# ug93tad/singa

Measured on AMD Instinct MI355X. Metric: images/sec (whole node) ResNet-50 bf16 training, higher is better.
Workload: dtype bf16; 1 GPU; model=ResNet-50, global_batch=1024, image=224, parallelism=dp1, exec=hipgraph, optimizer=SGD momentum 0.9 wd 1e-4, deterministic=True

## Files before the change

### singa_amd/autograd.py

```python
from __future__ import annotations

import builtins as _b
import math
import os
import sys
import threading
import types
import heapq
import weakref
from collections import Counter, deque
from typing import Callable, Dict, Iterator, List, Optional, Sequence, Tuple

import numpy as np
import torch

from . import memory as _mem
from . import tensor as _tensor
from .ops import functional as F
from .ops import glue as G
from .ops import native as N
from .tensor import Tensor

_TLS = threading.local()

# ... 790 lines not shown
            del dx._sg_absorbed
            dx = AccReplace(dx)
        elif acc is not None and (dx is acc or (isinstance(acc, F.LAZY_GRADS) and acc.value is not None
                                                and dx is acc.value)):
            dx = ACC_INPLACE
        res = [dx, ACCUMULATED if tgt is not None else dw]
        if self.has_bias:
            res.append(ACCUMULATED if tb is not None else db)
        return tuple(res)


class BatchNorm2d(Operator):

    def __init__(self, running_mean: torch.Tensor, running_var: torch.Tensor, momentum: float = 0.1,
                 eps: float = 1e-5, relu: bool = False, has_residual: bool = False, name=None,
                 colsum: bool = False):
        super().__init__(name)
        self.rm, self.rv = running_mean, running_var
        self.momentum, self.eps = momentum, eps
        self.relu, self.has_residual = relu, has_residual
        self.colsum = colsum

    def forward(self, x, gamma, beta, res=None):
        want = self.requires_grad and self.relu and (self.has_residual or (F.BN_WDOT and _training()))
        y, st = F.batchnorm_fwd(x, gamma, beta, self.rm, self.rv, _training(), self.momentum, self.eps, self.relu,
                                res, want_mask=want, want_colsum=self.colsum and self.requires_grad)
        if self.requires_grad:
            self.x, self.gamma, self.st = x, gamma, st
            self.beta = beta if F.BN_WDOT else None
            self.y = y if (want and st.mask is None) else None
        return y

    def backward(self, dy):
        tg, tb = self.grad_target(1), self.grad_target(2)
        dx, dg, db, dres = F.batchnorm_bwd(self.x, dy, self.gamma, self.st, self.y, need_dres=self.has_residual,
                                           relu=self.relu, dg_out=tg, db_out=tb, beta=getattr(self, "beta", None),
                                           lazy_dres=True)
        self.x = self.y = self.st = self.beta = None
        out = [dx, ACCUMULATED if tg is not None else dg, ACCUMULATED if tb is not None else db]
        if self.has_residual:
            out.append(dres)
# ... 31 lines not shown
        pre = getattr(dout, "_sg_gsum", None)
        if pre is not None and pre[1] is st.mask:
            g, gws = dout, pre[0]
            del dout._sg_gsum
        else:
            g, gws = F.bnres_masksum(dout, st.mask)
        prod = self.src[0][0] if self.src else None
        prod2 = None
        if (isinstance(prod, BatchNorm2d) and prod.relu and not prod.has_residual and F.BN_WDOT
                and getattr(prod, "st", None) is not None and prod.st.mask is not None
                and getattr(prod, "beta", None) is not None and (getattr(self, "sole", None) or {}).get(0, False)
                and self.needs_grad(0)):
            prod2 = (prod.st.mask, prod.gamma, prod.beta)
        tw, tg, tb = self.grad_target(1), self.grad_target(2), self.grad_target(3)
        cs = getattr(getattr(prod, "st", None), "colsum", None) if isinstance(prod, BatchNorm2d) else None
        dy, dw, dg, db = F.bnres_bwd(g, gws, y, w, st, gamma, dw_out=tw, dg_out=tg, db_out=tb, prod2=prod2, cs=cs)
        if tw is not None:
            _WGRAD_EPOCH[id(self.params[1])] = GRAD_EPOCH[0]
        g._sg_fresh = True
        acc = lambda tgt, v: ACCUMULATED if tgt is not None else v
        return dy, acc(tw, dw), acc(tg, dg), acc(tb, db), g


class ConvBNDualAddReLU(Operator):

    wants_sole = True

    def __init__(self, bn3, bnd, stride: int, name=None):
        super().__init__(name)
        self.p3 = (bn3.running_mean.data, bn3.running_var.data, 1.0 - bn3.momentum, bn3.eps)
        self.pd = (bnd.running_mean.data, bnd.running_var.data, 1.0 - bnd.momentum, bnd.eps)
# ... 31 lines not shown
        if pre is not None and pre[1] is st3.mask:
            g, gws = dout, pre[0]
            del dout._sg_gsum
        else:
            g, gws = F.bnres_masksum(dout, st3.mask)
        prod = self.src[0][0] if self.src else None
        prod2 = None
        if (isinstance(prod, BatchNorm2d) and prod.relu and not prod.has_residual and F.BN_WDOT
                and getattr(prod, "st", None) is not None and prod.st.mask is not None
                and getattr(prod, "beta", None) is not None and (getattr(self, "sole", None) or {}).get(0, False)
                and self.needs_grad(0)):
            prod2 = (prod.st.mask, prod.gamma, prod.beta)
        cs = getattr(getattr(prod, "st", None), "colsum", None) if isinstance(prod, BatchNorm2d) else None
        t = [self.grad_target(i) for i in (1, 2, 3, 5, 6, 7)]
        dy, dw3, dg3, db3 = F.bnres_bwd(g, gws, y, w3, st3, g3, dw_out=t[0], dg_out=t[1], db_out=t[2], prod2=prod2,
                                        cs=cs)
        dxs, dwd, dgd, dbd = F.bnres_bwd(g, gws, xs, wd, std, gd, dw_out=t[3], dg_out=t[4], db_out=t[5])
        for i, tg in ((1, t[0]), (5, t[3])):
            if tg is not None:
                _WGRAD_EPOCH[id(self.params[i])] = GRAD_EPOCH[0]
        dx = None
        if self.needs_grad(4):
            dx = dxs if self.stride == 1 else (F.StridedGrad(dxs, self.stride, xshape) if F.STRIDED_LAZY
                                               else F.strided_place(dxs, xshape, self.stride))
        acc = lambda tgt, v: ACCUMULATED if tgt is not None else v
        return (dy, acc(t[0], dw3), acc(t[1], dg3), acc(t[2], db3), dx, acc(t[3], dwd), acc(t[4], dgd),
                acc(t[5], dbd))


class DualBNAddReLU(Operator):

    def __init__(self, bn1, bn2, name=None):
# ... 1138 lines not shown
```

### singa_amd/csrc/bindings.cpp

```cpp
#include <hip/hip_runtime.h>
#include <pybind11/pybind11.h>
#include <pybind11/stl.h>
#include <stdint.h>
#include <stdexcept>
#include <string>
#include <vector>

namespace py = pybind11;
typedef uintptr_t P;
#define V(x) ((void*)(x))
#define CV(x) ((const void*)(x))
#define S(x) ((hipStream_t)(x))

extern "C" {
void sg_unary_fwd(int, const void*, void*, int64_t, int, float, hipStream_t);
void sg_unary_bwd(int, const void*, const void*, const void*, void*, int64_t, int, float, hipStream_t);
void sg_add_act(const void*, const void*, void*, int64_t, int, float, float, int, hipStream_t);
void sg_relu_bwd_from_y(const void*, const void*, void*, int64_t, int, hipStream_t);
void sg_mask_bits_apply(const void*, const void*, void*, int64_t, hipStream_t);
void sg_zero_ranges(void*, const void*, int, hipStream_t);
void sg_cast(const void*, int, void*, int, int64_t, hipStream_t);
void sg_dropout_fwd(const void*, void*, void*, int64_t, int, float, uint64_t, uint64_t, const void*, hipStream_t);
void sg_dropout_bwd(const void*, const void*, void*, int64_t, int, float, hipStream_t);
void sg_rand_fill(void*, int64_t, int, int, float, float, uint64_t, uint64_t, hipStream_t);
// ... 100 lines not shown
int sg_conv3x3_enabled();
void sg_bnres_wgrad(const void*, const void*, void*, int, int, int, hipStream_t);
void sg_bnres_dgrad(const void*, const void*, const void*, const void*, void*, int, int, int, void*, const void*,
                    hipStream_t);
void sg_bnres_coef(const void*, const void*, const void*, const void*, const void*, const void*, int, int, int, void*,
                   void*, void*, void*, void*, hipStream_t);
void sg_bnres_combine(const void*, const void*, const void*, const void*, int, const void*, const void*, int, int,
                      void*, void*, void*, void*, const void*, const void*, float, hipStream_t);
void sg_bnres_masksum(const void*, const void*, void*, void*, int64_t, int, hipStream_t);
void sg_set_dgrad_mask_out(int);
void sg_bn_apply_cs(const void*, const void*, const void*, void*, void*, void*, int64_t, int, int, hipStream_t);
void sg_conv_dgrad_gsum(const void*, const void*, void*, int, int, int, int, int, int, int, int, int, int, int, int,
                        int, int, int, void*, const void*, void*, const void*, int, int, int, hipStream_t);
int sg_sk_tail_ok(int, int, int);
void sg_bnres_gram_stats(const void*, const void*, const void*, int, int, int, void*, hipStream_t);
int sg_sk_tail2(const void*, const void*, const void*, const void*, const void*, void*, void*, int, int, int, int,
                hipStream_t);
void sg_bnres_fold(const void*, const void*, const void*, const void*, const void*, const void*, int, int, int, void*,
                   void*, void*, hipStream_t);
void sg_strided_pick(const void*, void*, int, int, int, int, int, int, int, int, hipStream_t);
int sg_sk_tail(const void*, const void*, void*, void*, const void*, const void*, const void*, void*, int, int, int, int,
               hipStream_t);
void sg_workq_set(int);
int sg_workq_enabled();
int sg_cu_count();
void sg_cu_hog(int, double, int, int*, hipStream_t);
int sg_fattn_ok(int, int);
int sg_fattn_fwd(const void*, void*, float*, const float*, int64_t, int, int, int, int, float, hipStream_t);
int sg_fattn_bwd(const void*, const void*, const void*, const float*, const float*, int64_t, void*, float*, int, int,
                 int, int, float, hipStream_t);
// ... 388 lines not shown
                              int sh, int sw, int ph, int pw, int dh, int dw, P wt, P acc, P bn_ws, P mask, int acc_s,
                              int acc_Ho, int acc_Wo, P s) {
    sg_conv_dgrad_gsum(CV(dy), CV(w), V(dx), N, H, W, C, K, R, Sd, Ho, Wo, sh, sw, ph, pw, dh, dw, V(wt), CV(acc),
                       V(bn_ws), CV(mask), acc_s, acc_Ho, acc_Wo, S(s));
    CHK("conv_dgrad_gsum");
  });
  m.def("strided_pick", [](P x, P y, int N, int H, int W, int C, int Ho, int Wo, int st, int place, P s) {
    sg_strided_pick(CV(x), V(y), N, H, W, C, Ho, Wo, st, place, S(s));
    CHK("strided_pick");
  });
  m.def("sk_tail_ok", [](int M, int N, int K) { return sg_sk_tail_ok(M, N, K); });
  m.def("bnres_gram_stats", [](P w, P gram, P cs, int cs_rows, int K4, int C, P ws, P s) {
    sg_bnres_gram_stats(CV(w), CV(gram), CV(cs), cs_rows, K4, C, V(ws), S(s));
    CHK("bnres_gram_stats");
  });
  m.def("sk_tail2", [](P y, P x, P wf, P shift, P ones, P out, P mask, int M, int N, int K1, int K2, P s) {
    const int r = sg_sk_tail2(CV(y), CV(x), CV(wf), CV(shift), CV(ones), V(out), V(mask), M, N, K1, K2, S(s));
    CHK("sk_tail2");
    return r;
  });
  m.def("bnres_fold", [](P w3, P wd, P s3, P f3, P sd, P fd, int N, int K1, int K2, P wf, P shift, P ones, P s) {
    sg_bnres_fold(CV(w3), CV(wd), CV(s3), CV(f3), CV(sd), CV(fd), N, K1, K2, V(wf), V(shift), V(ones), S(s));
    CHK("bnres_fold");
  });
  m.def("sk_tail", [](P a, P w, P out, P stats, P scale, P shift, P res, P mask, int M, int N, int K, int pass, P s) {
    const int r = sg_sk_tail(CV(a), CV(w), V(out), V(stats), CV(scale), CV(shift), CV(res), V(mask), M, N, K, pass,
                             S(s));
    CHK("sk_tail");
    return r;
  });
// ... 108 lines not shown
```

### singa_amd/csrc/kernels/bnres.hip

```cpp
#include <algorithm>
#include <stdexcept>

#include "igemm_kern.h"

namespace sg {
namespace bnres {

__global__ void __launch_bounds__(256) coef_k(const float* __restrict__ G, const bf16* __restrict__ w,
                                              const float* __restrict__ gws, const float* __restrict__ mean,
                                              const float* __restrict__ invstd, const float* __restrict__ gamma,
                                              float inv_p, int K4, int C, float* __restrict__ coef,
                                              float* __restrict__ wf, float* __restrict__ wu, float* __restrict__ dg,
                                              float* __restrict__ db) {
  const int lane = threadIdx.x & 63;
  const int k = blockIdx.x * 4 + (threadIdx.x >> 6);
  if (k >= K4) return;
  const bf16* wr = w + (int64_t)k * C;
  const float* gr = G + (int64_t)k * C;
  float sgc = 0.f;
  for (int c = lane; c < C; c += 64) {
    const float wv = (float)wr[c];
    sgc += wv * gr[c];
    wf[(int64_t)k * C + c] = wv;
  }
// ... 143 lines not shown
                                             const float* __restrict__ s3, const float* __restrict__ f3,
                                             const float* __restrict__ sd, const float* __restrict__ fd, int N,
                                             int K1, int K2, bf16* __restrict__ wf, float* __restrict__ shift,
                                             float* __restrict__ ones) {
  const int n = blockIdx.x;
  const int K = K1 + K2;
  for (int k = threadIdx.x; k < K; k += 256)
    wf[(int64_t)n * K + k] = k < K1 ? (bf16)(s3[n] * (float)w3[(int64_t)n * K1 + k])
                                    : (bf16)(sd[n] * (float)wd[(int64_t)n * K2 + k - K1]);
  if (threadIdx.x == 0) {
    shift[n] = f3[n] + fd[n];
    ones[n] = 1.f;
  }
}

__global__ void __launch_bounds__(256) gram_stats_k(const bf16* __restrict__ w, const float* __restrict__ gram,
                                                   const float* __restrict__ cs, int cs_rows, int K4, int C,
                                                   float* __restrict__ ws) {
  __shared__ float sh[8];
  const int k = blockIdx.x;
  const bf16* wk = w + (int64_t)k * C;
  float s1 = 0.f, s2 = 0.f;
  for (int i = threadIdx.x; i < C; i += 256) {
    const float* gi = gram + (int64_t)i * C;
    float t = 0.f;
    for (int j = 0; j < C; ++j) t += gi[j] * (float)wk[j];
    float ci = 0.f;
    for (int r = 0; r < cs_rows; ++r) ci += cs[(int64_t)r * C + i];
    const float wi = (float)wk[i];
    s1 += wi * ci;
    s2 += wi * t;
  }
  s1 = block_sum(s1, sh);
  s2 = block_sum(s2, sh);
  if (threadIdx.x == 0) {
    ws[k] = s1;
    ws[K4 + k] = s2;
  }
}

template <int BM, int BN, int AM, int BMODE, int OUT, int NTH, int WM, int WN, int STAGES>
void go(const GemmArgs& p, int tiles, int zdim, hipStream_t s) {
  constexpr int stages = STAGES * (BM + BN) * BK * 2;
  constexpr int rch = (STAGES == 1 || BM * (BN + 4) * 4 <= 152 * 1024) ? BM : BM / 4;
  constexpr int etile = OUT == OUT_BF16 ? rch * (BN + 4) * 4 : OUT == OUT_F32_ATOMIC ? BM * (BN + 4) * 4 : 0;
  constexpr int lds = stages > etile ? stages : etile;
  static_assert(lds <= 160 * 1024, "LDS budget");
  auto* kern = igemm_k<BM, BN, AM, BMODE, OUT, NTH, WM, WN, STAGES, 0>;
  if constexpr (lds > 65536) {
    static bool attr = [kern] {
      return hipFuncSetAttribute((const void*)kern, hipFuncAttributeMaxDynamicSharedMemorySize, lds) == hipSuccess;
    }();
// ... 11 lines not shown
}

}
}

using namespace sg;
using namespace sg::bnres;

extern "C" {

void sg_bnres_tune(int key, int v) {
  if (key == 0) g_wide = v;
  if (key == 1) g_dwide = v;
}

void sg_bnres_wgrad(const void* g, const void* y, void* out, int P, int K4, int C, hipStream_t s) {
  if ((K4 & 127) != 0 || (C & 63) != 0) throw std::runtime_error("bnres_wgrad: K4 % 128 and C % 64 required");
  GemmArgs p{};
  for (int i = 0; i < 16; ++i) {
    p.g.phs[i].dns = FastDiv(1);
    p.g.phs[i].dWp = FastDiv(1);
    p.g.phs[i].dHpWp = FastDiv(1);
  }
  p.M = K4 + C; p.N = C; p.K = P;
  p.a = (const bf16*)g; p.lda = K4; p.a_bytes = extent((int64_t)P * K4);
  p.a2 = (const bf16*)y; p.lda2 = C; p.a2_bytes = extent((int64_t)P * C); p.a2_split = K4;
  p.b = (const bf16*)y; p.ldb = C; p.b_bytes = p.a2_bytes;
  p.c = out; p.ldc = C; p.alpha = 1.f;
  const int nkt = (P + BK - 1) / BK;
  if (C >= 128 && (K4 & 255) == 0 && g_wide) {
    const int tiles = ((p.M + 255) / 256) * ((C + 127) / 128);
    const int slots = sg_cu_count();
    int sp = 1;
    long best = -1;
    for (int s2 = 1; s2 <= 256 && nkt / s2 >= 16; ++s2) {
      const long cost = (long)((tiles * s2 + slots - 1) / slots) * ((nkt + s2 - 1) / s2 + 6);
      if (best < 0 || cost < best) {
        best = cost;
        sp = s2;
// ... 6 lines not shown
  if (C >= 128) {
    const int tiles = ((p.M + 127) / 128) * ((C + 127) / 128);
    int sp = 1;
    while (tiles * sp < 512 && sp * 2 * 4 <= nkt) sp *= 2;
    p.k_per_split = ((nkt + sp - 1) / sp) * BK;
    go<128, 128, LM_KOUTER2, LM_KOUTER, OUT_F32_ATOMIC, 512, 2, 4, 2>(p, tiles, sp, s);
  } else {
    const int tiles = (p.M + 127) / 128;
    int sp = 1;
    while (tiles * sp < 768 && sp * 2 * 8 <= nkt) sp *= 2;
    p.k_per_split = ((nkt + sp - 1) / sp) * BK;
    go<128, 64, LM_KOUTER2, LM_KOUTER, OUT_F32_ATOMIC, 256, 2, 2, 2>(p, tiles, sp, s);
  }
}

void sg_bnres_dgrad(const void* g, const void* y, const void* bd, const void* bias, void* dx, int P, int K4, int C,
                    void* stats, const void* mask, hipStream_t s) {
  if ((K4 & 63) != 0 || (C & 63) != 0) throw std::runtime_error("bnres_dgrad: K4 % 64 and C % 64 required");
  GemmArgs p{};
  for (int i = 0; i < 16; ++i) {
    p.g.phs[i].dns = FastDiv(1);
    p.g.phs[i].dWp = FastDiv(1);
    p.g.phs[i].dHpWp = FastDiv(1);
  }
  p.M = P; p.N = C; p.K = K4 + C;
  p.a = (const bf16*)g; p.lda = K4; p.a_bytes = extent((int64_t)P * K4);
  p.a2 = (const bf16*)y; p.lda2 = C; p.a2_bytes = extent((int64_t)P * C); p.a2_split = K4;
  p.b = (const bf16*)bd; p.ldb = K4 + C; p.b_bytes = extent((int64_t)C * (K4 + C));
  p.c = dx; p.ldc = C; p.alpha = 1.f; p.beta = 0.f; p.bias = (const float*)bias;
  p.k_per_split = ((p.K + BK - 1) / BK) * BK;
// ... 56 lines not shown
                       (unsigned)(C / 8), (unsigned)W, (unsigned)H, (unsigned)Wo, (unsigned)Ho, (unsigned)st);
  else
    hipLaunchKernelGGL(pick_k, dim3(blocks), dim3(256), 0, s, (const uint4*)x, (uint4*)y, (unsigned)total,
                       (unsigned)(C / 8), (unsigned)Wo, (unsigned)Ho, (unsigned)W, (unsigned)H, (unsigned)st);
}

void sg_bnres_fold(const void* w3, const void* wd, const void* s3, const void* f3, const void* sd, const void* fd, int N,
                   int K1, int K2, void* wf, void* shift, void* ones, hipStream_t s) {
  hipLaunchKernelGGL(fold_k, dim3(N), dim3(256), 0, s, (const bf16*)w3, (const bf16*)wd, (const float*)s3,
                     (const float*)f3, (const float*)sd, (const float*)fd, N, K1, K2, (bf16*)wf, (float*)shift,
                     (float*)ones);
}

void sg_bnres_gram_stats(const void* w, const void* gram, const void* cs, int cs_rows, int K4, int C, void* ws,
                         hipStream_t s) {
  hipLaunchKernelGGL(gram_stats_k, dim3(K4), dim3(256), 0, s, (const bf16*)w, (const float*)gram, (const float*)cs,
                     cs_rows, K4, C, (float*)ws);
}

}
```

### singa_amd/layer.py

```python
from __future__ import annotations

import math
from collections import OrderedDict
from typing import Dict, List, Optional, Sequence, Tuple, Union

import numpy as np
import torch

from . import autograd
from .ops import glue as G
from . import device as _dev
from .tensor import Tensor


def _pair(v) -> Tuple[int, int]:
    if isinstance(v, (list, tuple)):
        return (int(v[0]), int(v[1]))
    return (int(v), int(v))


class Layer:
    sep = "."

    def __init__(self):
# ... 240 lines not shown
        self.momentum = momentum
        self.eps = eps

    def initialize(self, x, *args, **kwargs):
        C = x.shape[1]
        dev = x.device
        s = _new_param((C,), dev)
        G.fill_(s.data, 1.0)
        self._param("scale", s, wd_mult=0.0)
        self._param("bias", _new_param((C,), dev), wd_mult=0.0)
        self._state("running_mean", Tensor((C,), dev, requires_grad=False))
        rv = Tensor((C,), dev, requires_grad=False)
        G.fill_(rv.data, 1.0)
        self._state("running_var", rv)

    def forward(self, x, relu: bool = False, residual: Optional[Tensor] = None, colsum: bool = False):
        op = autograd.BatchNorm2d(self.running_mean.data, self.running_var.data, 1.0 - self.momentum, self.eps,
                                  relu=relu, has_residual=residual is not None, colsum=colsum)
        if residual is not None:
            return op(x, self.scale, self.bias, residual)
        return op(x, self.scale, self.bias)


class LayerNorm(Layer):
    def __init__(self, eps=1e-5):
        super().__init__()
        self.eps = eps

    def initialize(self, x):
        D = x.shape[-1]
        g = _new_param((D,), x.device)
        G.fill_(g.data, 1.0)
        self._param("scale", g, wd_mult=0.0)
# ... 266 lines not shown
```

### singa_amd/models/resnet.py

```python
from __future__ import annotations

import os
from types import SimpleNamespace
from typing import List, Sequence

import torch

from .. import memory as _mem
from .. import autograd, layer, model
from ..ops import functional as F
from ..ops import native as N
from ..tensor import Tensor
from ..ops import glue as G


class InputPrep(autograd.Operator):

    def __init__(self, dtype=torch.bfloat16, name=None):
        super().__init__(name)
        self.dtype = dtype

    def forward(self, x):
        if x.is_cuda and x.dim() == 4:
            C = x.shape[1]
# ... 132 lines not shown
        self.conv1 = layer.Conv2d(planes, 1, bias=False)
        self.bn1 = layer.BatchNorm2d()
        self.conv2 = layer.Conv2d(planes, 3, stride=stride, padding=1, bias=False)
        self.bn2 = layer.BatchNorm2d()
        self.conv3 = layer.Conv2d(planes * self.expansion, 1, bias=False)
        self.bn3 = layer.BatchNorm2d()
        self.has_down = downsample
        if downsample:
            self.down_conv = layer.Conv2d(planes * self.expansion, 1, stride=stride, bias=False)
            self.down_bn = layer.BatchNorm2d()
        _feeds_bn(self.conv1, self.conv2, self.conv3, *([self.down_conv] if downsample else []))

    def forward(self, x):
        out = self.bn1(self.conv1(x), relu=True)
        tail = autograd.training and F.BNRES and x.data.is_cuda and not autograd._TRACE
        out = self.bn2(self.conv2(out), relu=True, colsum=tail)
        c3 = self.conv3
        if self.has_down:
            dc = self.down_conv
            if (tail and os.environ.get("SINGA_FUSED_DOWN_TAIL", "1") != "0" and c3.kernel_size == (1, 1) and c3.stride == (1, 1) and tuple(c3.padding) == (0, 0)
                    and not c3.bias and c3.group == 1 and dc.kernel_size == (1, 1) and tuple(dc.padding) == (0, 0)
                    and dc.stride[0] == dc.stride[1] and not dc.bias and dc.group == 1
                    and F.bnres_ok(out.data, (c3.nb_kernels, out.shape[1], 1, 1), None, down=(x.data, dc.stride[0]))):
                k4 = SimpleNamespace(shape=(1, c3.nb_kernels), device=x.device)
                for lyr, t in ((dc, x), (c3, out), (self.down_bn, k4), (self.bn3, k4)):
                    if not lyr._initialized:
                        lyr.initialize(t)
                        lyr._initialized = True
                b3, bd = self.bn3, self.down_bn
                return autograd.ConvBNDualAddReLU(b3, bd, dc.stride[0])(out, c3.W, b3.scale, b3.bias, x, dc.W,
                                                                        bd.scale, bd.bias)
# ... 111 lines not shown
```

### singa_amd/ops/functional.py

```python
from __future__ import annotations

import math
import os
import threading
from typing import Optional, Sequence, Tuple

import numpy as np
import torch
import torch.nn.functional as F

from .. import memory as _mem
from . import cpu as CP
from . import glue as G
from . import native as N

UNARY = {"relu": 0, "sigmoid": 1, "tanh": 2, "stanh": 3, "gelu": 4, "identity": 5, "softplus": 6, "square": 7,
         "abs": 8, "exp": 9, "leakyrelu": 10, "elu": 11, "selu": 12, "gelu_tanh": 13, "sqrt": 14, "neg": 15,
         "reciprocal": 16, "log": 17, "sign": 18, "erf": 19, "cos": 20, "sin": 21, "tan": 22, "cosh": 23,
         "sinh": 24, "acos": 25, "asin": 26, "atan": 27, "acosh": 28, "asinh": 29, "atanh": 30, "ceil": 31,
         "floor": 32, "round": 33, "softsign": 34, "scale": 35, "adds": 36, "rsqrt": 37, "pows": 38}

_CPU_UNARY = {
    "relu": torch.relu, "sigmoid": torch.sigmoid, "tanh": torch.tanh,
    "stanh": lambda x: 1.7159047 * torch.tanh(0.66666667 * x),
# ... 1302 lines not shown
    _no_native("colsum", x2)
    if CP.ok(x2, out):
        s0 = G.reduce(x2, [0], "sum")
        if out is not None:
            s0 = G.binary("add", out, s0, out=out)
        return s0, (G.reduce(x2, [0], "sumsq") if with_sq else None)
    xf = x2.float()
    s0 = xf.sum(0)
    if out is not None:
        out.add_(s0)
        s0 = out
    return s0, ((xf * xf).sum(0) if with_sq else None)


class BNState:
    __slots__ = ("mean", "invstd", "scale", "shift", "mask", "colsum")

    def __init__(self, mean, invstd, scale, shift, mask=None):
        self.mean, self.invstd, self.scale, self.shift, self.mask = mean, invstd, scale, shift, mask
        self.colsum = None


LAZY_RES = os.environ.get("SINGA_AMD_LAZY_RES", "1") != "0"


class MaskedGrad:

    _sg_fresh = True

    def __init__(self, g: torch.Tensor, mask: torch.Tensor):
        self.g, self.mask, self.value = g, mask, None
        self.shape, self.dtype, self.device = g.shape, g.dtype, g.device

    def is_floating_point(self) -> bool:
        return True
# ... 97 lines not shown
        dx = _like(x)
        N.lib().bn_bwd_pool(x.data_ptr(), dyc.data_ptr(), arg.data_ptr(), st.scale.data_ptr(), st.shift.data_ptr(),
                            st.mean.data_ptr(), st.invstd.data_ptr(), gamma.data_ptr(), _ws(R, C, x.device).data_ptr(),
                            coef.data_ptr(), dg.data_ptr(), db.data_ptr(), dx.data_ptr(), Nn, H, W, C, Ho, Wo,
                            kernel[0], kernel[1], stride[0], stride[1], padding[0], padding[1], N.stream())
        dx._sg_fresh = True
        return dx, dg, db
    dpre = pool2d_bwd(x.shape, x, dy, arg, kernel, stride, padding, True)
    dx, dg, db, _ = batchnorm_bwd(x, dpre, gamma, st, None, need_dres=False, relu=True, dg_out=dg_out, db_out=db_out)
    return dx, dg, db


def batchnorm_fwd(x: torch.Tensor, gamma: torch.Tensor, beta: torch.Tensor, run_mean: torch.Tensor,
                  run_var: torch.Tensor, training: bool, momentum: float = 0.1, eps: float = 1e-5,
                  relu: bool = False, residual: Optional[torch.Tensor] = None, want_mask: bool = False,
                  want_colsum: bool = False):
    C = x.shape[1]
    if _bn_native(x):
        L = N.lib()
        R = x.numel() // C
        dev = x.device
        mean, invstd, scale, shift = _bn_params(x, gamma, beta, run_mean, run_var, training, momentum, eps)
        res = None
        if residual is not None:
            res = residual
            if res.dtype != x.dtype or not _same_layout(res, x):
                res = G.to(res, x.dtype, torch.channels_last if x.dim() == 4 else torch.contiguous_format)
        y = _like(x)
        mask = None
        if want_mask and relu and C % 8 == 0:
            mask = _mem.empty(R * C // 8, dtype=torch.uint8, device=dev)
        if want_colsum and res is None and x.dtype == torch.bfloat16 and C % 64 == 0:
            cs = _zeros32(32 * C, dev)
            L.bn_apply_cs(x.data_ptr(), scale.data_ptr(), shift.data_ptr(), y.data_ptr(), N.ptr(mask), cs.data_ptr(),
                          R, C, int(relu), N.stream())
            st = BNState(mean, invstd, scale, shift, mask)
            st.colsum = cs
            y._sg_cs_slots = cs
            return y, st
        L.bn_apply(x.data_ptr(), scale.data_ptr(), shift.data_ptr(), N.ptr(res), y.data_ptr(), R, C, int(relu),
                   N.dt(x), N.stream(), N.ptr(mask))
        return y, BNState(mean, invstd, scale, shift, mask)
    _no_native("batchnorm_fwd", x)
    if (CP.ok(x, gamma, beta, run_mean, run_var, residual) and run_mean.is_contiguous() and run_var.is_contiguous()
            and x.dim() in (2, 4)):
        xc = CP.dense32(x)
        Nn = x.shape[0]
        HW = x.numel() // (Nn * C) if Nn * C else 0
        y = _mem.empty(x.shape, dtype=torch.float32)
        mean = _mem.empty(C, dtype=torch.float32)
        invstd = _mem.empty(C, dtype=torch.float32)
# ... 79 lines not shown
    ok = (BNRES and _native_ok(y) and y.dtype == torch.bfloat16 and N.is_cl(y) and y.dim() == 4
          and tuple(w_shape[2:]) == (1, 1) and y.shape[1] == C and C % 64 == 0 and K4 % 128 == 0
          and not N.lib().deterministic() and y.numel() // C * K4 * 2 < (1 << 31))
    if not ok:
        return False
    if down is not None:
        x, s = down
        return (_native_ok(x) and x.dtype == torch.bfloat16 and x.dim() == 4 and N.is_cl(x) and x.shape[1] % 64 == 0
                and x.shape[0] == y.shape[0] and (x.shape[2] - 1) // s + 1 == y.shape[2]
                and (x.shape[3] - 1) // s + 1 == y.shape[3] and x.numel() * 2 < (1 << 31))
    return res is not None and tuple(res.shape) == (y.shape[0], K4, y.shape[2], y.shape[3])


TAIL_RECOMPUTE = os.environ.get("SINGA_AMD_TAIL_RECOMPUTE", "1") != "0"
GRAM_STATS = os.environ.get("SINGA_AMD_GRAM_STATS", "1") != "0"


def tail_stats_ws(a: torch.Tensor, w: torch.Tensor, M: int, C: int, K4: int):
    L = N.lib()
    dev = a.device
    if not GRAM_STATS:
        ws = zeroed_ws(32 * 2 * K4, dev)
        L.sk_tail(a.data_ptr(), w.data_ptr(), 0, ws.data_ptr(), 0, 0, 0, 0, M, K4, C, 0, N.stream())
        return ws, 32
    gram = _zeros32(C * C, dev)
    L.bnres_wgrad(0, a.data_ptr(), gram.data_ptr(), M, 0, C, N.stream())
    cs = getattr(a, "_sg_cs_slots", None)
    if cs is None or cs.numel() % C != 0:
        cs = colsum(a.permute(0, 2, 3, 1).reshape(M, C))[0]
    ws = _mem.empty(2 * K4, dtype=torch.float32, device=dev)
    L.bnres_gram_stats(w.data_ptr(), gram.data_ptr(), cs.data_ptr(), cs.numel() // C, K4, C, ws.data_ptr(),
                       N.stream())
    return ws, 1


def bnres_fwd(y: torch.Tensor, w: torch.Tensor, gamma, beta, run_mean, run_var, training: bool, momentum: float,
              eps: float, res: torch.Tensor):
    if not (TAIL_RECOMPUTE and training and _native_ok(y, w) and y.dtype == torch.bfloat16 and y.dim() == 4
            and N.is_cl(y) and tuple(w.shape[2:]) == (1, 1) and res is not None and res.dtype == torch.bfloat16
            and N.is_cl(res)):
        return None
    if not (w.dtype == torch.bfloat16 and N.is_cl(w)):
        w = G.to(w, torch.bfloat16, torch.channels_last)
    Nn, C, H, W = y.shape
    K = w.shape[0]
    M = Nn * H * W
    L = N.lib()
# ... 77 lines not shown
    return t


def bnres_masksum(dy: torch.Tensor, mask: torch.Tensor):
    if dy.dtype != torch.bfloat16 or not N.is_cl(dy):
        dy = G.to(dy, torch.bfloat16, torch.channels_last)
    C = dy.shape[1]
    R = dy.numel() // C
    g = _like(dy)
    ws = _zeros32(32 * 2 * C, dy.device)
    N.lib().bnres_masksum(dy.data_ptr(), mask.data_ptr(), g.data_ptr(), ws.data_ptr(), R, C, N.stream())
    return g, ws


def bnres_bwd(g: torch.Tensor, gws: torch.Tensor, y: torch.Tensor, w: torch.Tensor, st: "BNState",
              gamma: torch.Tensor, dw_out=None, dg_out=None, db_out=None, prod2=None, cs=None):
    L = N.lib()
    s = N.stream()
    dev = g.device
    Nn, K4, H, W = g.shape
    C = y.shape[1]
    P = Nn * H * W
    f32 = torch.float32
    wb = w if (w.dtype == torch.bfloat16 and (N.is_cl(w) or w.is_contiguous())) else G.to(w, torch.bfloat16)
    aug = _zeros32((K4 + C) * C, dev)
    L.bnres_wgrad(g.data_ptr(), y.data_ptr(), aug.data_ptr(), P, K4, C, s)
    Gm, Gram = aug[:K4 * C], aug[K4 * C:]
    coef = _mem.empty(3 * K4, dtype=f32, device=dev)
    wf = _mem.empty(K4 * C, dtype=f32, device=dev)
    wu = _mem.empty(K4 * C, dtype=f32, device=dev)
    dg = dg_out if dg_out is not None else _zeros32(K4, dev)
    db = db_out if db_out is not None else _zeros32(K4, dev)
    L.bnres_coef(Gm.data_ptr(), wb.data_ptr(), gws.data_ptr(), st.mean.data_ptr(), st.invstd.data_ptr(),
                 gamma.data_ptr(), P, K4, C, coef.data_ptr(), wf.data_ptr(), wu.data_ptr(), dg.data_ptr(),
                 db.data_ptr(), s)
    TM = _zeros32(K4 * C + C * C, dev)
    T, Mm = TM[:K4 * C], TM[K4 * C:]
    L.ggemm(0, wf.data_ptr(), C, 0, 0, Gram.data_ptr(), C, 1, 0, T.data_ptr(), C, 0, K4, C, C, 1.0, 1.0, 0, 0, 2, 0,
            1, 0, 0, 0, 0, s)
    L.ggemm(0, wf.data_ptr(), C, 1, 0, wu.data_ptr(), C, 1, 0, Mm.data_ptr(), C, 0, C, C, K4, 1.0, 1.0, 0, 0, 2, 0,
            1, 0, 0, 0, 0, s)
    if cs is None:
# ... 472 lines not shown
```

Measured before the change: 16530 images/s.

## Fuse Gram accumulation into BN apply and reuse forward Gram in tail backward

Adds a bn_apply_gram kernel that computes the channel Gram matrix (upper triangle, via MFMA) while applying BN+ReLU and the column sums. The forward tail statistics then use it through a triangular gram_stats variant that also mirrors the matrix to full. The Gram matrix from the forward tail-stats step is attached to the activation and reused in bnres_bwd, so the backward wgrad GEMM computes only the K4 rows and not the extra C rows. The fused forward path is disabled in deterministic mode because it uses atomics; the backward reuse still applies there. The cost is keeping a small C×C float buffer alive until backward.

```diff
diff --git a/singa_amd/autograd.py b/singa_amd/autograd.py
--- a/singa_amd/autograd.py
+++ b/singa_amd/autograd.py
@@ -828,17 +828,19 @@
 
     def __init__(self, running_mean: torch.Tensor, running_var: torch.Tensor, momentum: float = 0.1,
                  eps: float = 1e-5, relu: bool = False, has_residual: bool = False, name=None,
-                 colsum: bool = False):
+                 colsum: bool = False, gram: Optional[bool] = None):
         super().__init__(name)
         self.rm, self.rv = running_mean, running_var
         self.momentum, self.eps = momentum, eps
         self.relu, self.has_residual = relu, has_residual
         self.colsum = colsum
+        self.gram = colsum if gram is None else (gram and colsum)
 
     def forward(self, x, gamma, beta, res=None):
         want = self.requires_grad and self.relu and (self.has_residual or (F.BN_WDOT and _training()))
         y, st = F.batchnorm_fwd(x, gamma, beta, self.rm, self.rv, _training(), self.momentum, self.eps, self.relu,
-                                res, want_mask=want, want_colsum=self.colsum and self.requires_grad)
+                                res, want_mask=want, want_colsum=self.colsum and self.requires_grad,
+                                want_gram=self.gram and self.requires_grad and _training())
         if self.requires_grad:
             self.x, self.gamma, self.st = x, gamma, st
             self.beta = beta if F.BN_WDOT else None
@@ -900,7 +902,8 @@
             prod2 = (prod.st.mask, prod.gamma, prod.beta)
         tw, tg, tb = self.grad_target(1), self.grad_target(2), self.grad_target(3)
         cs = getattr(getattr(prod, "st", None), "colsum", None) if isinstance(prod, BatchNorm2d) else None
-        dy, dw, dg, db = F.bnres_bwd(g, gws, y, w, st, gamma, dw_out=tw, dg_out=tg, db_out=tb, prod2=prod2, cs=cs)
+        dy, dw, dg, db = F.bnres_bwd(g, gws, y, w, st, gamma, dw_out=tw, dg_out=tg, db_out=tb, prod2=prod2, cs=cs,
+                                     gram=getattr(y, "_sg_gram_full", None))
         if tw is not None:
             _WGRAD_EPOCH[id(self.params[1])] = GRAD_EPOCH[0]
         g._sg_fresh = True
@@ -962,8 +965,9 @@
         cs = getattr(getattr(prod, "st", None), "colsum", None) if isinstance(prod, BatchNorm2d) else None
         t = [self.grad_target(i) for i in (1, 2, 3, 5, 6, 7)]
         dy, dw3, dg3, db3 = F.bnres_bwd(g, gws, y, w3, st3, g3, dw_out=t[0], dg_out=t[1], db_out=t[2], prod2=prod2,
-                                        cs=cs)
-        dxs, dwd, dgd, dbd = F.bnres_bwd(g, gws, xs, wd, std, gd, dw_out=t[3], dg_out=t[4], db_out=t[5])
+                                        cs=cs, gram=getattr(y, "_sg_gram_full", None))
+        dxs, dwd, dgd, dbd = F.bnres_bwd(g, gws, xs, wd, std, gd, dw_out=t[3], dg_out=t[4], db_out=t[5],
+                                         gram=getattr(xs, "_sg_gram_full", None))
         for i, tg in ((1, t[0]), (5, t[3])):
             if tg is not None:
                 _WGRAD_EPOCH[id(self.params[i])] = GRAD_EPOCH[0]
diff --git a/singa_amd/csrc/bindings.cpp b/singa_amd/csrc/bindings.cpp
--- a/singa_amd/csrc/bindings.cpp
+++ b/singa_amd/csrc/bindings.cpp
@@ -138,6 +138,10 @@
                         int, int, int, void*, const void*, void*, const void*, int, int, int, hipStream_t);
 int sg_sk_tail_ok(int, int, int);
 void sg_bnres_gram_stats(const void*, const void*, const void*, int, int, int, void*, hipStream_t);
+void sg_bnres_gram_stats_tri(const void*, void*, const void*, int, int, int, void*, hipStream_t);
+void sg_bnres_wgrad_g(const void*, const void*, void*, int, int, int, hipStream_t);
+void sg_bn_apply_gram(const void*, const void*, const void*, void*, void*, void*, void*, int64_t, int, int,
+                      hipStream_t);
 int sg_sk_tail2(const void*, const void*, const void*, const void*, const void*, void*, void*, int, int, int, int,
                 hipStream_t);
 void sg_bnres_fold(const void*, const void*, const void*, const void*, const void*, const void*, int, int, int, void*,
@@ -556,6 +560,18 @@
     sg_bnres_gram_stats(CV(w), CV(gram), CV(cs), cs_rows, K4, C, V(ws), S(s));
     CHK("bnres_gram_stats");
   });
+  m.def("bnres_gram_stats_tri", [](P w, P gram, P cs, int cs_rows, int K4, int C, P ws, P s) {
+    sg_bnres_gram_stats_tri(CV(w), V(gram), CV(cs), cs_rows, K4, C, V(ws), S(s));
+    CHK("bnres_gram_stats_tri");
+  });
+  m.def("bnres_wgrad_g", [](P g, P y, P out, int Pn, int K4, int C, P s) {
+    sg_bnres_wgrad_g(CV(g), CV(y), V(out), Pn, K4, C, S(s));
+    CHK("bnres_wgrad_g");
+  });
+  m.def("bn_apply_gram", [](P x, P scale, P shift, P y, P mask, P colsum, P gram, int64_t R, int C, int relu, P s) {
+    sg_bn_apply_gram(CV(x), CV(scale), CV(shift), V(y), V(mask), V(colsum), V(gram), R, C, relu, S(s));
+    CHK("bn_apply_gram");
+  });
   m.def("sk_tail2", [](P y, P x, P wf, P shift, P ones, P out, P mask, int M, int N, int K1, int K2, P s) {
     const int r = sg_sk_tail2(CV(y), CV(x), CV(wf), CV(shift), CV(ones), V(out), V(mask), M, N, K1, K2, S(s));
     CHK("sk_tail2");
diff --git a/singa_amd/csrc/kernels/bnres.hip b/singa_amd/csrc/kernels/bnres.hip
--- a/singa_amd/csrc/kernels/bnres.hip
+++ b/singa_amd/csrc/kernels/bnres.hip
@@ -181,28 +181,198 @@
   }
 }
 
-__global__ void __launch_bounds__(256) gram_stats_k(const bf16* __restrict__ w, const float* __restrict__ gram,
+__global__ void __launch_bounds__(256) gram_stats_k(const bf16* __restrict__ w, float* __restrict__ gram,
                                                    const float* __restrict__ cs, int cs_rows, int K4, int C,
-                                                   float* __restrict__ ws) {
+                                                   float* __restrict__ ws, int tri) {
   __shared__ float sh[8];
   const int k = blockIdx.x;
   const bf16* wk = w + (int64_t)k * C;
   float s1 = 0.f, s2 = 0.f;
+  if (tri) {
+    for (int e = threadIdx.x; e < C * C; e += 256) {
+      const int i = e / C, j = e - i * C;
+      if (j >= i) s2 += (j > i ? 2.f : 1.f) * (float)wk[i] * (float)wk[j] * gram[e];
+    }
+  }
   for (int i = threadIdx.x; i < C; i += 256) {
-    const float* gi = gram + (int64_t)i * C;
-    float t = 0.f;
-    for (int j = 0; j < C; ++j) t += gi[j] * (float)wk[j];
     float ci = 0.f;
     for (int r = 0; r < cs_rows; ++r) ci += cs[(int64_t)r * C + i];
     const float wi = (float)wk[i];
     s1 += wi * ci;
-    s2 += wi * t;
+    if (!tri) {
+      const float* gi = gram + (int64_t)i * C;
+      float t = 0.f;
+      for (int j = 0; j < C; ++j) t += gi[j] * (float)wk[j];
+      s2 += wi * t;
+    }
   }
   s1 = block_sum(s1, sh);
   s2 = block_sum(s2, sh);
   if (threadIdx.x == 0) {
     ws[k] = s1;
     ws[K4 + k] = s2;
+  }
+  if (tri) {
+    const int per = (C * C + (int)gridDim.x - 1) / (int)gridDim.x;
+    const int e1 = min(C * C, (k + 1) * per);
+    for (int e = k * per + threadIdx.x; e < e1; e += 256) {
+      const int i = e / C, j = e - i * C;
+      if (j < i) gram[e] = gram[(int64_t)j * C + i];
+    }
+  }
+}
+
+template <int C>
+__global__ void __launch_bounds__(256) bn_apply_gram_k(const bf16* __restrict__ x, const float* __restrict__ scale,
+                                                      const float* __restrict__ shift, bf16* __restrict__ y,
+                                                      uint8_t* __restrict__ mask, float* __restrict__ colsum,
+                                                      float* __restrict__ gram, int64_t R, int relu, int64_t rpw) {
+  constexpr int CPR = C / 8;
+  constexpr int RPP = 256 / CPR;
+  constexpr int BR = 128;
+  constexpr int UR = BR / RPP;
+  constexpr int IMG = BR * C * 2;
+  constexpr int T = C / 16, NS = T + 1, KG = 4 / (T / 2);
+  constexpr int LDS_BYTES = 2 * IMG > C * C * 4 ? 2 * IMG : C * C * 4;
+  static_assert(C == 64 || C == 128, "C");
+  static_assert(256 * 8 * 4 <= LDS_BYTES, "column-sum scratch");
+  __shared__ __attribute__((aligned(16))) char lds[LDS_BYTES];
+  typedef short v4s __attribute__((ext_vector_type(4)));
+
+  const int t = threadIdx.x;
+  const int ch = t % CPR, rl = t / CPR;
+  const int c0 = ch * 8;
+  const int l = t & 63;
+  const int wv = __builtin_amdgcn_readfirstlane(t >> 6);
+  const int pr = wv % (T / 2), kg = wv / (T / 2);
+
+  float sc[8], sf[8], csum[8];
+  ldc<8>(scale + c0, sc);
+  ldc<8>(shift + c0, sf);
+#pragma unroll
+  for (int k = 0; k < 8; ++k) csum[k] = 0.f;
+
+  int oa0[NS], oa1[NS], ob0[NS], ob1[NS];
+  {
+    const int g = l >> 4, i = l & 15, q = i >> 2, pp = i & 3;
+    const int kb0 = 8 * g + q, kb1 = kb0 + 4;
+#pragma unroll
+    for (int s = 0; s < NS; ++s) {
+      const int ti = s < T - pr ? pr : T - 1 - pr;
+      const int tj = s < T - pr ? pr + s : T - 1 - pr + s - (T - pr);
+      const int ca = ti * 16 + 4 * pp, cb = tj * 16 + 4 * pp;
+      oa0[s] = kb0 * (C * 2) + kouter_swz<C>(kb0, ca >> 3) * 16 + (ca & 7) * 2;
+      oa1[s] = kb1 * (C * 2) + kouter_swz<C>(kb1, ca >> 3) * 16 + (ca & 7) * 2;
+      ob0[s] = kb0 * (C * 2) + kouter_swz<C>(kb0, cb >> 3) * 16 + (cb & 7) * 2;
+      ob1[s] = kb1 * (C * 2) + kouter_swz<C>(kb1, cb >> 3) * 16 + (cb & 7) * 2;
+    }
+  }
+  f32x4 acc[NS];
+#pragma unroll
+  for (int s = 0; s < NS; ++s) acc[s] = f32x4{0.f, 0.f, 0.f, 0.f};
+
+  const int64_t r0 = (int64_t)blockIdx.x * rpw;
+  const int64_t rend = r0 + rpw < R ? r0 + rpw : R;
+  const int nblk = (int)((rend - r0 + BR - 1) / BR);
+
+  bf16x8 raw[UR];
+  auto load = [&](int b) {
+#pragma unroll
+    for (int u = 0; u < UR; ++u) {
+      const int64_t r = r0 + (int64_t)b * BR + rl + RPP * u;
+      bf16x8 z;
+#pragma unroll
+      for (int k = 0; k < 8; ++k) z[k] = (bf16)0.f;
+      raw[u] = r < rend ? __builtin_nontemporal_load((const bf16x8*)(x + r * C + c0)) : z;
+    }
+  };
+  auto apply = [&](int b, char* img) {
+#pragma unroll
+    for (int u = 0; u < UR; ++u) {
+      const int row = rl + RPP * u;
+      const int64_t r = r0 + (int64_t)b * BR + row;
+      bf16x8 o;
+#pragma unroll
+      for (int k = 0; k < 8; ++k) o[k] = (bf16)0.f;
+      if (r < rend) {
+        unsigned bits = 0;
+#pragma unroll
+        for (int k = 0; k < 8; ++k) {
+          float v = (float)raw[u][k] * sc[k] + sf[k] + 0.f;
+          if (relu) v = fmaxf(v, 0.f);
+          o[k] = (bf16)v;
+          csum[k] += (float)o[k];
+          bits |= ((float)o[k] > 0.f ? 1u : 0u) << k;
+        }
+        const int64_t off = r * C + c0;
+        __builtin_nontemporal_store(o, (bf16x8*)(y + off));
+        if (mask) mask[off >> 3] = (uint8_t)bits;
+      }
+      *(bf16x8*)(img + row * (C * 2) + kouter_swz<C>(row, ch) * 16) = o;
+    }
+  };
+  auto frag = [&](const char* img, int o0, int o1) {
+    v4s x0 = __builtin_amdgcn_ds_read_tr16_b64_v4i16((__attribute__((address_space(3))) v4s*)(img + o0));
+    v4s x1 = __builtin_amdgcn_ds_read_tr16_b64_v4i16((__attribute__((address_space(3))) v4s*)(img + o1));
+    i16x8 r;
+    r[0] = x0[0]; r[1] = x0[1]; r[2] = x0[2]; r[3] = x0[3];
+    r[4] = x1[0]; r[5] = x1[1]; r[6] = x1[2]; r[7] = x1[3];
+    return __builtin_bit_cast(bf16x8, r);
+  };
+
+  if (nblk > 0) {
+    load(0);
+    apply(0, lds);
+  }
+  lds_barrier(0);
+  for (int b = 0; b < nblk; ++b) {
+    const bool more = b + 1 < nblk;
+    if (more) load(b + 1);
+    const char* img = lds + (b & 1) * IMG;
+#pragma unroll
+    for (int kk = KG == 1 ? 0 : kg; kk < BR / 32; kk += KG) {
+      const char* ik = img + kk * 32 * (C * 2);
+#pragma unroll
+      for (int s = 0; s < NS; ++s) {
+        const bf16x8 fa = frag(ik, oa0[s], oa1[s]);
+        const bf16x8 fb = frag(ik, ob0[s], ob1[s]);
+        acc[s] = __builtin_amdgcn_mfma_f32_16x16x32_bf16(fa, fb, acc[s], 0, 0, 0);
+      }
+    }
+    if (more) apply(b + 1, lds + ((b + 1) & 1) * IMG);
+    lds_barrier(0);
+  }
+
+  float* red = (float*)lds;
+#pragma unroll
+  for (int k = 0; k < 8; ++k) red[t * 8 + k] = csum[k];
+  lds_barrier(0);
+  if (t < C) {
+    float a = 0.f;
+    for (int q = 0; q < RPP; ++q) a += red[(q * CPR + t / 8) * 8 + (t % 8)];
+    atomicAdd(colsum + (int64_t)(blockIdx.x & 31) * C + t, a);
+  }
+  lds_barrier(0);
+  float* gt = (float*)lds;
+#pragma unroll
+  for (int round = 0; round < KG; ++round) {
+    if (kg == round) {
+#pragma unroll
+      for (int s = 0; s < NS; ++s) {
+        const int ti = s < T - pr ? pr : T - 1 - pr;
+        const int tj = s < T - pr ? pr + s : T - 1 - pr + s - (T - pr);
+#pragma unroll
+        for (int r = 0; r < 4; ++r) {
+          float* e = gt + (ti * 16 + 4 * (l >> 4) + r) * C + tj * 16 + (l & 15);
+          *e = round == 0 ? acc[s][r] : *e + acc[s][r];
+        }
+      }
+    }
+    lds_barrier(0);
+  }
+  for (int seg = wv; seg < C * (C / 64); seg += 4) {
+    const int i = seg / (C / 64), j = (seg % (C / 64)) * 64 + l;
+    if (j >= (i & ~15)) atomicAdd(gram + i * C + j, gt[i * C + j]);
   }
 }
 
@@ -244,7 +414,8 @@
   if (key == 1) g_dwide = v;
 }
 
-void sg_bnres_wgrad(const void* g, const void* y, void* out, int P, int K4, int C, hipStream_t s) {
+static void wgrad_launch(const void* g, const void* y, void* out, int P, int K4, int C, bool with_gram,
+                         hipStream_t s) {
   if ((K4 & 127) != 0 || (C & 63) != 0) throw std::runtime_error("bnres_wgrad: K4 % 128 and C % 64 required");
   GemmArgs p{};
   for (int i = 0; i < 16; ++i) {
@@ -252,7 +423,7 @@
     p.g.phs[i].dWp = FastDiv(1);
     p.g.phs[i].dHpWp = FastDiv(1);
   }
-  p.M = K4 + C; p.N = C; p.K = P;
+  p.M = K4 + (with_gram ? C : 0); p.N = C; p.K = P;
   p.a = (const bf16*)g; p.lda = K4; p.a_bytes = extent((int64_t)P * K4);
   p.a2 = (const bf16*)y; p.lda2 = C; p.a2_bytes = extent((int64_t)P * C); p.a2_split = K4;
   p.b = (const bf16*)y; p.ldb = C; p.b_bytes = p.a2_bytes;
@@ -289,6 +460,15 @@
   }
 }
 
+void sg_bnres_wgrad(const void* g, const void* y, void* out, int P, int K4, int C, hipStream_t s) {
+  wgrad_launch(g, y, out, P, K4, C, true, s);
+}
+
+void sg_bnres_wgrad_g(const void* g, const void* y, void* out, int P, int K4, int C, hipStream_t s) {
+  if (K4 <= 0) throw std::runtime_error("bnres_wgrad_g: K4 > 0 required");
+  wgrad_launch(g, y, out, P, K4, C, false, s);
+}
+
 void sg_bnres_dgrad(const void* g, const void* y, const void* bd, const void* bias, void* dx, int P, int K4, int C,
                     void* stats, const void* mask, hipStream_t s) {
   if ((K4 & 63) != 0 || (C & 63) != 0) throw std::runtime_error("bnres_dgrad: K4 % 64 and C % 64 required");
@@ -375,8 +555,29 @@
 
 void sg_bnres_gram_stats(const void* w, const void* gram, const void* cs, int cs_rows, int K4, int C, void* ws,
                          hipStream_t s) {
-  hipLaunchKernelGGL(gram_stats_k, dim3(K4), dim3(256), 0, s, (const bf16*)w, (const float*)gram, (const float*)cs,
-                     cs_rows, K4, C, (float*)ws);
-}
-
-}
+  hipLaunchKernelGGL(gram_stats_k, dim3(K4), dim3(256), 0, s, (const bf16*)w, (float*)const_cast<void*>(gram),
+                     (const float*)cs, cs_rows, K4, C, (float*)ws, 0);
+}
+
+void sg_bn_apply_gram(const void* x, const void* scale, const void* shift, void* y, void* mask, void* colsum,
+                      void* gram, int64_t R, int C, int relu, hipStream_t s) {
+  if (C != 64 && C != 128) throw std::runtime_error("bn_apply_gram: C = 64 or 128 required");
+  if (R <= 0) return;
+  const int64_t target = (int64_t)sg_cu_count() * (C == 64 ? 4 : 2);
+  int64_t rpw = ((R + target - 1) / target + 127) / 128 * 128;
+  const unsigned grid = (unsigned)((R + rpw - 1) / rpw);
+  if (C == 64)
+    hipLaunchKernelGGL(bn_apply_gram_k<64>, dim3(grid), dim3(256), 0, s, (const bf16*)x, (const float*)scale,
+                       (const float*)shift, (bf16*)y, (uint8_t*)mask, (float*)colsum, (float*)gram, R, relu, rpw);
+  else
+    hipLaunchKernelGGL(bn_apply_gram_k<128>, dim3(grid), dim3(256), 0, s, (const bf16*)x, (const float*)scale,
+                       (const float*)shift, (bf16*)y, (uint8_t*)mask, (float*)colsum, (float*)gram, R, relu, rpw);
+}
+
+void sg_bnres_gram_stats_tri(const void* w, void* gram, const void* cs, int cs_rows, int K4, int C, void* ws,
+                             hipStream_t s) {
+  hipLaunchKernelGGL(gram_stats_k, dim3(K4), dim3(256), 0, s, (const bf16*)w, (float*)gram, (const float*)cs, cs_rows,
+                     K4, C, (float*)ws, 1);
+}
+
+}
diff --git a/singa_amd/layer.py b/singa_amd/layer.py
--- a/singa_amd/layer.py
+++ b/singa_amd/layer.py
@@ -278,9 +278,11 @@
         G.fill_(rv.data, 1.0)
         self._state("running_var", rv)
 
-    def forward(self, x, relu: bool = False, residual: Optional[Tensor] = None, colsum: bool = False):
+    def forward(self, x, relu: bool = False, residual: Optional[Tensor] = None, colsum: bool = False,
+                gram: Optional[bool] = None):
         op = autograd.BatchNorm2d(self.running_mean.data, self.running_var.data, 1.0 - self.momentum, self.eps,
-                                  relu=relu, has_residual=residual is not None, colsum=colsum)
+                                  relu=relu, has_residual=residual is not None, colsum=colsum,
+                                  gram=colsum if gram is None else gram)
         if residual is not None:
             return op(x, self.scale, self.bias, residual)
         return op(x, self.scale, self.bias)
diff --git a/singa_amd/models/resnet.py b/singa_amd/models/resnet.py
--- a/singa_amd/models/resnet.py
+++ b/singa_amd/models/resnet.py
@@ -170,7 +170,8 @@
     def forward(self, x):
         out = self.bn1(self.conv1(x), relu=True)
         tail = autograd.training and F.BNRES and x.data.is_cuda and not autograd._TRACE
-        out = self.bn2(self.conv2(out), relu=True, colsum=tail)
+        strided = self.has_down and tuple(self.down_conv.stride) != (1, 1)
+        out = self.bn2(self.conv2(out), relu=True, colsum=tail, gram=tail and not strided)
         c3 = self.conv3
         if self.has_down:
             dc = self.down_conv
diff --git a/singa_amd/ops/functional.py b/singa_amd/ops/functional.py
--- a/singa_amd/ops/functional.py
+++ b/singa_amd/ops/functional.py
@@ -1340,11 +1340,12 @@
 
 
 class BNState:
-    __slots__ = ("mean", "invstd", "scale", "shift", "mask", "colsum")
+    __slots__ = ("mean", "invstd", "scale", "shift", "mask", "colsum", "gram")
 
     def __init__(self, mean, invstd, scale, shift, mask=None):
         self.mean, self.invstd, self.scale, self.shift, self.mask = mean, invstd, scale, shift, mask
         self.colsum = None
+        self.gram = None
 
 
 LAZY_RES = os.environ.get("SINGA_AMD_LAZY_RES", "1") != "0"
@@ -1472,7 +1473,7 @@
 def batchnorm_fwd(x: torch.Tensor, gamma: torch.Tensor, beta: torch.Tensor, run_mean: torch.Tensor,
                   run_var: torch.Tensor, training: bool, momentum: float = 0.1, eps: float = 1e-5,
                   relu: bool = False, residual: Optional[torch.Tensor] = None, want_mask: bool = False,
-                  want_colsum: bool = False):
+                  want_colsum: bool = False, want_gram: bool = False):
     C = x.shape[1]
     if _bn_native(x):
         L = N.lib()
@@ -1490,9 +1491,16 @@
             mask = _mem.empty(R * C // 8, dtype=torch.uint8, device=dev)
         if want_colsum and res is None and x.dtype == torch.bfloat16 and C % 64 == 0:
             cs = _zeros32(32 * C, dev)
-            L.bn_apply_cs(x.data_ptr(), scale.data_ptr(), shift.data_ptr(), y.data_ptr(), N.ptr(mask), cs.data_ptr(),
-                          R, C, int(relu), N.stream())
             st = BNState(mean, invstd, scale, shift, mask)
+            if want_gram and APPLY_GRAM and C in (64, 128) and not L.deterministic():
+                gram = _zeros32(C * C, dev)
+                L.bn_apply_gram(x.data_ptr(), scale.data_ptr(), shift.data_ptr(), y.data_ptr(), N.ptr(mask),
+                                cs.data_ptr(), gram.data_ptr(), R, C, int(relu), N.stream())
+                st.gram = gram
+                y._sg_gram = gram
+            else:
+                L.bn_apply_cs(x.data_ptr(), scale.data_ptr(), shift.data_ptr(), y.data_ptr(), N.ptr(mask),
+                              cs.data_ptr(), R, C, int(relu), N.stream())
             st.colsum = cs
             y._sg_cs_slots = cs
             return y, st
@@ -1602,6 +1610,8 @@
 
 TAIL_RECOMPUTE = os.environ.get("SINGA_AMD_TAIL_RECOMPUTE", "1") != "0"
 GRAM_STATS = os.environ.get("SINGA_AMD_GRAM_STATS", "1") != "0"
+APPLY_GRAM = os.environ.get("SINGA_AMD_APPLY_GRAM", "1") != "0" and GRAM_STATS
+BWD_GRAM = os.environ.get("SINGA_AMD_TAIL_BWD_GRAM", "1") != "0"
 
 
 def tail_stats_ws(a: torch.Tensor, w: torch.Tensor, M: int, C: int, K4: int):
@@ -1611,14 +1621,20 @@
         ws = zeroed_ws(32 * 2 * K4, dev)
         L.sk_tail(a.data_ptr(), w.data_ptr(), 0, ws.data_ptr(), 0, 0, 0, 0, M, K4, C, 0, N.stream())
         return ws, 32
-    gram = _zeros32(C * C, dev)
-    L.bnres_wgrad(0, a.data_ptr(), gram.data_ptr(), M, 0, C, N.stream())
+    gram = getattr(a, "_sg_gram", None)
+    tri = gram is not None and gram.numel() == C * C
+    if tri:
+        del a._sg_gram
+    else:
+        gram = _zeros32(C * C, dev)
+        L.bnres_wgrad(0, a.data_ptr(), gram.data_ptr(), M, 0, C, N.stream())
     cs = getattr(a, "_sg_cs_slots", None)
     if cs is None or cs.numel() % C != 0:
         cs = colsum(a.permute(0, 2, 3, 1).reshape(M, C))[0]
     ws = _mem.empty(2 * K4, dtype=torch.float32, device=dev)
-    L.bnres_gram_stats(w.data_ptr(), gram.data_ptr(), cs.data_ptr(), cs.numel() // C, K4, C, ws.data_ptr(),
-                       N.stream())
+    (L.bnres_gram_stats_tri if tri else L.bnres_gram_stats)(w.data_ptr(), gram.data_ptr(), cs.data_ptr(),
+                                                            cs.numel() // C, K4, C, ws.data_ptr(), N.stream())
+    a._sg_gram_full = gram
     return ws, 1
 
 
@@ -1726,7 +1742,7 @@
 
 
 def bnres_bwd(g: torch.Tensor, gws: torch.Tensor, y: torch.Tensor, w: torch.Tensor, st: "BNState",
-              gamma: torch.Tensor, dw_out=None, dg_out=None, db_out=None, prod2=None, cs=None):
+              gamma: torch.Tensor, dw_out=None, dg_out=None, db_out=None, prod2=None, cs=None, gram=None):
     L = N.lib()
     s = N.stream()
     dev = g.device
@@ -1735,9 +1751,13 @@
     P = Nn * H * W
     f32 = torch.float32
     wb = w if (w.dtype == torch.bfloat16 and (N.is_cl(w) or w.is_contiguous())) else G.to(w, torch.bfloat16)
-    aug = _zeros32((K4 + C) * C, dev)
-    L.bnres_wgrad(g.data_ptr(), y.data_ptr(), aug.data_ptr(), P, K4, C, s)
-    Gm, Gram = aug[:K4 * C], aug[K4 * C:]
+    if gram is not None and BWD_GRAM and gram.numel() == C * C:
+        Gm, Gram = _zeros32(K4 * C, dev), gram
+        L.bnres_wgrad_g(g.data_ptr(), y.data_ptr(), Gm.data_ptr(), P, K4, C, s)
+    else:
+        aug = _zeros32((K4 + C) * C, dev)
+        L.bnres_wgrad(g.data_ptr(), y.data_ptr(), aug.data_ptr(), P, K4, C, s)
+        Gm, Gram = aug[:K4 * C], aug[K4 * C:]
     coef = _mem.empty(3 * K4, dtype=f32, device=dev)
     wf = _mem.empty(K4 * C, dtype=f32, device=dev)
     wu = _mem.empty(K4 * C, dtype=f32, device=dev)
```

Result: no change. 16650 images/s, median of 6 (+0.7%).
